# QuantEcon/dynamic_factor_models

Measured on NVIDIA H100. Metric: EM iters/sec (N=200,r=8,T=500), higher is better.
Workload: dtype f64

## Files before the change

### dynamic_factor_models_b200/csrc/dfm_kernels_fused2.cuh

```cuda
#pragma once
#include <algorithm>
#include "dfm_kernels_fused.cuh"
#ifdef DFM_EMU
struct CUtensorMap { char opaque[128]; };
#define DFM_GRID_CONSTANT
#else
#include <cuda.h>
#define DFM_GRID_CONSTANT __grid_constant__
#endif

namespace dfm {

#ifndef F2_SBS
#define F2_SBS 1
#endif
#ifndef F2_S
#define F2_S (3 / F2_SBS)
#endif
#define F2_STG (F2_SBS * 8 * F2_TS)
#ifndef F2_TC
#define F2_TC 172
#endif
#define F2_TS F2_TC
#define F2_NCW 6
#define F2_GPARTS_S 4
#define F2_GPARTS ((R == 8) ? (F2_NCW + 1) : F2_GPARTS_S)
#define F2_NRB (((F2_TC + 7) / 8 + F2_NCW - 1) / F2_NCW)
#define F2_NKC (((F2_TC + 3) / 4 + F2_NCW - 1) / F2_NCW)
static_assert(F2_TC % 16 == 4 || F2_TC % 16 == 12, "ring pitch must be 4 or 12 mod 16");
static_assert(F2_TC <= 256 && (F2_TC * 64) % 128 == 0, "TMA box / stage alignment");
#define F2_NEXS(R_) ((F2_S * F2_STG - 4 * (R_) * (R_)) / FUSED_SCR(R_))
#define F2_RTAIL(R_) (F2_S * F2_STG - 4 * (R_) * (R_))
#ifndef F2_L2WIN_PCT
#define F2_L2WIN_PCT 67
#endif

#ifndef DFM_EMU
__device__ __forceinline__ uint32_t f2_smem_u32(const void* p) { return (uint32_t)__cvta_generic_to_shared(p); }
__device__ __forceinline__ void f2_mbar_init(uint64_t* bar, int cnt) { asm volatile("mbarrier.init.shared::cta.b64 [%0], %1;" ::"r"(f2_smem_u32(bar)), "r"(cnt)); }
__device__ __forceinline__ void f2_mbar_expect(uint64_t* bar, uint32_t bytes) { asm volatile("mbarrier.arrive.expect_tx.shared::cta.b64 _, [%0], %1;" ::"r"(f2_smem_u32(bar)), "r"(bytes) : "memory"); }
__device__ __forceinline__ void f2_mbar_arrive(uint64_t* bar) { asm volatile("mbarrier.arrive.shared::cta.b64 _, [%0];" ::"r"(f2_smem_u32(bar)) : "memory"); }
__device__ __forceinline__ void f2_mbar_wait(uint64_t* bar, uint32_t phase) {
  asm volatile("{\n.reg .pred p;\nWAIT_%=:\nmbarrier.try_wait.parity.shared::cta.b64 p, [%0], %1;\n@p bra DONE_%=;\nbra WAIT_%=;\nDONE_%=:\n}" ::"r"(f2_smem_u32(bar)), "r"(phase) : "memory");
}
__device__ __forceinline__ void f2_tma_2d(void* dst, const CUtensorMap* tmap, int x, int y, uint64_t* bar, uint64_t policy) {
  asm volatile("cp.async.bulk.tensor.2d.shared::cluster.global.mbarrier::complete_tx::bytes.L2::cache_hint [%0], [%1, {%2, %3}], [%4], %5;"
               ::"r"(f2_smem_u32(dst)), "l"(reinterpret_cast<uint64_t>(tmap)), "r"(x), "r"(y), "r"(f2_smem_u32(bar)), "l"(policy) : "memory");
}

__device__ __forceinline__ int f2_round_win(const int* win, int B, int b) {
  const int G = (int)gridDim.x;
  return (b / G < B / G) ? win[0] : win[1];
}
#endif


#ifndef DFM_EMU
struct F2Ring {
  double* ring; uint64_t* full; uint64_t* empty;
  int rs; uint32_t rph; bool wrap;
  __device__ __forceinline__ void advance() { if (++rs == F2_S) { rs = 0; rph ^= 1; wrap = true; } }
  __device__ __forceinline__ void skip(long long n) { for (long long q = 0; q < n; ++q) advance(); }
};

__device__ __forceinline__ void f2_produce(F2Ring& rg, const CUtensorMap* tmap, int row0, int T, int N, bool c_outer, const int* win) {
  const int lane = threadIdx.x & 31;
  const int nsb = (N + 8 * F2_SBS - 1) / (8 * F2_SBS), nck = (T + F2_TC - 1) / F2_TC;
  const int n_out = c_outer ? nck : nsb, n_in = c_outer ? nsb : nck, nw = *win;
  const int wc = c_outer ? nck - 1 : 0, w0 = c_outer ? nsb - nw : 0, w1 = c_outer ? nsb : nw;
  uint64_t pol_win, pol_first;
  asm volatile("createpolicy.fractional.L2::evict_normal.b64 %0, 1.0;" : "=l"(pol_win));
  asm volatile("createpolicy.fractional.L2::evict_first.b64 %0, 1.0;" : "=l"(pol_first));
  for (int o = 0; o < n_out; ++o)
    for (int i = 0; i < n_in; ++i) {
      const int c = c_outer ? o : i, sb = c_outer ? i : nsb - 1 - o;
      if (rg.wrap) f2_mbar_wait(&rg.empty[rg.rs], rg.rph ^ 1);
      if (lane == 0) {
        f2_mbar_expect(&rg.full[rg.rs], (uint32_t)(F2_STG * 8));
        f2_tma_2d(rg.ring + (size_t)rg.rs * F2_STG, tmap, c * F2_TC, row0 + sb * 8 * F2_SBS, &rg.full[rg.rs],
                  (c == wc && sb >= w0 && sb < w1) ? pol_win : pol_first);
      }
      __syncwarp();
      rg.advance();
    }
}

template <int R>
__device__ __forceinline__ double f2_consume_E(F2Ring& rg, int cw, int T, int N, int Tp, int Np, double* Z, const double* Lam,
                                               const double* rinv) {
  const int lane = threadIdx.x & 31, lr = lane >> 2, lc = lane & 3;
  const int nsg = (N + 8 * F2_SBS - 1) / (8 * F2_SBS), nck = (T + F2_TC - 1) / F2_TC;
  double qacc = 0.0;
  for (int c = 0; c < nck; ++c) {
    const int len = (T - c * F2_TC < F2_TC) ? T - c * F2_TC : F2_TC;
    double d[F2_NRB][2][2];
#pragma unroll
    for (int j = 0; j < F2_NRB; ++j) { d[j][0][0] = 0.0; d[j][0][1] = 0.0; d[j][1][0] = 0.0; d[j][1][1] = 0.0; }
    for (int sg = 0; sg < nsg; ++sg) {
      f2_mbar_wait(&rg.full[rg.rs], rg.rph);
      const double* stage = rg.ring + (size_t)rg.rs * F2_STG;
#pragma unroll
      for (int sub = 0; sub < F2_SBS; ++sub) {
        const double* tile = stage + (size_t)sub * 8 * F2_TS;
        const int sb = sg * F2_SBS + sub;
        double rn[2], lm[2], av[2][F2_NRB];
#pragma unroll
        for (int kc = 0; kc < 2; ++kc) {
          const int n = sb * 8 + kc * 4 + lc;
          const bool nok = n < N;
          rn[kc] = nok ? (rinv ? rinv[n] : 1.0) : 0.0;
          lm[kc] = (nok && lr < R) ? Lam[LI(n, lr)] : 0.0;
          const double* trow = tile + (kc * 4 + lc) * F2_TS + lr;
#pragma unroll
          for (int j = 0; j < F2_NRB; ++j) {
            const int t0 = (cw + j * F2_NCW) * 8;
            av[kc][j] = (nok && t0 + lr < len) ? trow[t0] : 0.0;
          }
        }
#pragma unroll
        for (int kc = 0; kc < 2; ++kc)
#pragma unroll
          for (int j = 0; j < F2_NRB; ++j) {
            const double ar = av[kc][j] * rn[kc];
            qacc += av[kc][j] * ar;
            asm volatile("mma.sync.aligned.m8n8k4.row.col.f64.f64.f64.f64 {%0,%1}, {%2}, {%3}, {%0,%1};\n"
                         : "+d"(d[j][kc][0]), "+d"(d[j][kc][1]) : "d"(ar), "d"(lm[kc]));
          }
      }
      __syncwarp();
      if (lane == 0) f2_mbar_arrive(&rg.empty[rg.rs]);
      rg.advance();
    }
#pragma unroll
    for (int j = 0; j < F2_NRB; ++j) {
      const int tl = (cw + j * F2_NCW) * 8 + lr;
      if (tl < len) { const int t = c * F2_TC + tl; Z[ZI(t, 2 * lc)] = d[j][0][0] + d[j][1][0]; Z[ZI(t, 2 * lc + 1)] = d[j][0][1] + d[j][1][1]; }
    }
  }
  return qacc;
}

template <int R>
__device__ __forceinline__ void f2_consume_M(F2Ring& rg, int cw, int T, int N, int Tp, int Np, const double* Z, double* Lam,
                                             double* sxx, double* part) {
  const int lane = threadIdx.x & 31, lr = lane >> 2, lc = lane & 3;
  const int nsg = (N + 8 * F2_SBS - 1) / (8 * F2_SBS), nck = (T + F2_TC - 1) / F2_TC;
  double d[F2_SBS][F2_NKC][2], s2[F2_SBS];
#pragma unroll
  for (int sub = 0; sub < F2_SBS; ++sub) {
    s2[sub] = 0.0;
#pragma unroll
    for (int j = 0; j < F2_NKC; ++j) { d[sub][j][0] = 0.0; d[sub][j][1] = 0.0; }
  }
  for (int sg = nsg - 1; sg >= 0; --sg)
    for (int c = 0; c < nck; ++c) {
      f2_mbar_wait(&rg.full[rg.rs], rg.rph);
      const double* stage = rg.ring + (size_t)rg.rs * F2_STG;
      const int len = (T - c * F2_TC < F2_TC) ? T - c * F2_TC : F2_TC;
      const double* zc = Z + (size_t)lr * Tp + c * F2_TC + lc;
      double bv[F2_NKC];
#pragma unroll
      for (int j = 0; j < F2_NKC; ++j) { const int t0 = (cw + j * F2_NCW) * 4; bv[j] = (t0 + lc < len) ? zc[t0] : 0.0; }
#pragma unroll
      for (int sub = 0; sub < F2_SBS; ++sub) {
        const bool nok = (sg * F2_SBS + sub) * 8 + lr < N;
        const double* trow = stage + (size_t)sub * 8 * F2_TS + lr * F2_TS + lc;
        double av[F2_NKC];
#pragma unroll
        for (int j = 0; j < F2_NKC; ++j) { const int t0 = (cw + j * F2_NCW) * 4; av[j] = (nok && t0 + lc < len) ? trow[t0] : 0.0; }
#pragma unroll
        for (int j = 0; j < F2_NKC; ++j) {
          s2[sub] += av[j] * av[j];
          asm volatile("mma.sync.aligned.m8n8k4.row.col.f64.f64.f64.f64 {%0,%1}, {%2}, {%3}, {%0,%1};\n"
                       : "+d"(d[sub][j][0]), "+d"(d[sub][j][1]) : "d"(av[j]), "d"(bv[j]));
        }
      }
      __syncwarp();
      if (lane == 0) f2_mbar_arrive(&rg.empty[rg.rs]);
      rg.advance();
      if (c == nck - 1) {
#pragma unroll
        for (int sub = 0; sub < F2_SBS; ++sub) {
          const int sb = sg * F2_SBS + sub;
          double sq = s2[sub];
          sq += __shfl_xor_sync(0xffffffffu, sq, 1); sq += __shfl_xor_sync(0xffffffffu, sq, 2);
          double* pb = part + (size_t)(sb & 1) * F2_NCW * 72 + cw * 72;
          double t0_ = 0.0, t1_ = 0.0;
#pragma unroll
          for (int j = 0; j < F2_NKC; ++j) { t0_ += d[sub][j][0]; t1_ += d[sub][j][1]; d[sub][j][0] = 0.0; d[sub][j][1] = 0.0; }
          pb[2 * lane] = t0_; pb[2 * lane + 1] = t1_;
          if (lc == 0) pb[64 + lr] = sq;
          asm volatile("bar.sync 1, %0;" ::"n"(F2_NCW * 32) : "memory");
          const int ct = cw * 32 + lane;
          if (ct < 72) {
            const double* pp_ = part + (size_t)(sb & 1) * F2_NCW * 72 + ct;
            double tot_ = 0.0;
#pragma unroll
            for (int w_ = 0; w_ < F2_NCW; ++w_) tot_ += pp_[w_ * 72];
            if (ct < 64) {
              const int l_ = ct >> 1, h_ = ct & 1, row = l_ >> 2, col = 2 * (l_ & 3) + h_, n = sb * 8 + row;
              if (n < N && col < R) Lam[LI(n, col)] = tot_;
            } else { const int n = sb * 8 + (ct - 64); if (n < N) sxx[n] = tot_; }
          }
          s2[sub] = 0.0;
        }
      }
    }
}
#endif

#define F2_PNT_GPU ((F2_NCW + 1) * 32)
#ifdef DFM_EMU
#define F2_PSYNC() ((void)0)
#define F2_PTID 0
#define F2_PNT 1
#else
#define F2_PSYNC() asm volatile("bar.sync 2, %0;" ::"n"(F2_PNT_GPU) : "memory")
// ... 4 lines not shown
#define DFM_FUSED2_BOUNDS
#else
#define DFM_FUSED2_BOUNDS __launch_bounds__(256, 2)
#endif
template <int R>
__global__ void DFM_FUSED2_BOUNDS k_em_fused2(FusedArgs a, const DFM_GRID_CONSTANT CUtensorMap tmap) {
  DFM_SMEM(sm);
  constexpr int RR = R * R, NP = R * (R + 1) / 2;
  const int T = a.T, N = a.N;
  const int Tp = pad4mod16(T), Np = pad4mod16(N);
  double* Z = sm;
  double* Lam = Z + (size_t)FZ * Tp;
  double* rinv = Lam + (size_t)R * Np;
  double* Rv = rinv + N;
  double* sxx = Rv + N;
  double* mats = sxx + N;
  double* M = mats;            double* Q = M + RR;        double* C = Q + RR;        double* Pp = C + RR;
  double* Pi = Pp + RR;        double* Pf = Pi + RR;      double* Wm = Pf + RR;      double* G = Wm + RR;
  double* Phi = G + RR;        double* Jm = Phi + RR;     double* Pn = Jm + RR;      double* T1 = Pn + RR;
  double* T2 = T1 + RR;        double* Ps = T2 + RR;      double* Psn = Ps + RR;     double* SPall = Psn + RR;
  double* SP00 = SPall + RR;   double* SPff2 = SP00 + RR; double* SP11 = SPff2 + RR; double* Sm = SP11 + RR;
  double* S11m = Sm + RR;      double* Pfinf = S11m + RR; double* Phinf = Pfinf + RR; double* Jinf = Phinf + RR;
  double* Winf = Jinf + RR;    double* Ppinf = Winf + RR; double* IJM = Ppinf + RR;  double* Pfprev = IJM + RR;
  double* tmp = Pfprev + RR;
  double* red = tmp + 2 * R;
  double* scal = red + 40;
  int* ctl = (int*)(scal + 8);
  double* bnd = scal + 16;
  double* part = bnd;
  double* ring = bnd + (((size_t)97 * R + RR > 2 * F2_NCW * 72) ? (size_t)97 * R + RR : 2 * F2_NCW * 72);
#ifndef DFM_EMU
  ring += ((128u - (f2_smem_u32(ring) & 127u)) & 127u) / 8;
#endif
  double* gscr = a.scratch + (size_t)DFM_BX * T * FUSED_SCR(R);
#define GSC(t_) (gscr + (size_t)(t_) * FUSED_SCR(R))
#define SCRP(t_) (((t_) < F2_NEXS(R)) ? (ring + (size_t)(t_) * FUSED_SCR(R)) : (gscr + (size_t)(t_) * FUSED_SCR(R)))
#define GPS(t_) (gscr + (size_t)(t_) * FUSED_SCR(R) + 4 * RR)
#ifndef DFM_EMU
  __shared__ uint64_t fullb[F2_S], emptyb[F2_S];
  if (threadIdx.x == 0) { for (int s_ = 0; s_ < F2_S; ++s_) { f2_mbar_init(&fullb[s_], 1); f2_mbar_init(&emptyb[s_], F2_NCW); } }
  asm volatile("fence.mbarrier_init.release.cluster;" ::: "memory");
  __syncthreads();
  F2Ring rg; rg.ring = ring; rg.full = fullb; rg.empty = emptyb; rg.rs = 0; rg.rph = 0; rg.wrap = false;
#endif
  const double eps = 1e-14;

  for (int b = DFM_BX; b < a.B; b += DFM_GX) {
#ifdef DFM_EMU
    const double* X = a.X + (size_t)b * T * N;
#endif
#ifndef DFM_EMU
    if (a.ready) {
      if (threadIdx.x == 0) {
        const int* f_ = a.ready + b / a.ready_chunk; int v_ = 0;
        for (;;) { asm volatile("ld.acquire.sys.global.s32 %0, [%1];" : "=r"(v_) : "l"(f_) : "memory"); if (v_) break; __nanosleep(256); }
      }
      __syncthreads();
    }
#endif
// ... 108 lines not shown
            w_gemm<R>(T1, Pf, false, M, true);
            w_gemm<R>(Jinf, T1, false, Pi, false);
            break;
          }
          if (frozen_at < 0 && dmax <= eps * pmax) frozen_at = t;
          for (int e = DFM_LANE; e < RR; e += DFM_WSZ) Pp[e] = Pn[e];
          DFM_WSYNC();
          ++t;
        }
        const int frozen = nE < T;
        if (DFM_LANE == 0) { ctl[0] = nE; ctl[3] = frozen; }
        if (frozen) {
          w_gemm<R>(IJM, Jinf, false, M, false);
          for (int e = DFM_LANE; e < RR; e += DFM_WSZ) { int i = e / R, j = e % R; IJM[e] = ((i == j) ? 1.0 : 0.0) - IJM[e]; }
          DFM_WSYNC();
          const int n3 = T - (nE > 0 ? nE : 1), n5 = (T - 2) - (nE - 1) + 1;
          if (n3 > 0) {
            w_matpow<R>(Phi, Phinf, blk_chunk_len(n3, F2_PNT_GPU / 8), T1, T2);
            w_gemm<R>(Pp, Phi, false, Phi, false); w_gemm<R>(Pi, Pp, false, Pp, false);
            w_gemm<R>(Pf, Pi, false, Pi, false);   w_gemm<R>(Jm, Pf, false, Pf, false);
          }
          if (n5 > 0) {
            w_matpow<R>(Pn, Jinf, blk_chunk_len(n5, F2_PNT_GPU / 8), T1, T2);
            double* gl_ = GSC(T - 1);
            w_gemm<R>(T1, Pn, false, Pn, false);
            for (int e = DFM_LANE; e < RR; e += DFM_WSZ) gl_[e] = T1[e];
            w_gemm<R>(T2, T1, false, T1, false);
            for (int e = DFM_LANE; e < RR; e += DFM_WSZ) gl_[RR + e] = T2[e];
            w_gemm<R>(T1, T2, false, T2, false);
            for (int e = DFM_LANE; e < RR; e += DFM_WSZ) gl_[2 * RR + e] = T1[e];
            w_gemm<R>(T2, T1, false, T1, false);
            for (int e = DFM_LANE; e < RR; e += DFM_WSZ) gl_[3 * RR + e] = T2[e];
            DFM_WSYNC();
          }
        }
        DFM_WSYNC();
      };
      auto chain_bwd = [&]() {
        const int nE = ctl[0], frozen = ctl[3];
        int t;
        for (int e = DFM_LANE; e < RR; e += DFM_WSZ) {
          double v = frozen ? Pfinf[e] : (GSC(T - 1))[e];
          Psn[e] = v; SPall[e] = v; SPff2[e] = v; SP00[e] = 0.0; SP11[e] = 0.0;
          GPS(T - 1)[e] = v;
        }
        DFM_WSYNC();
        const int lo = frozen ? nE - 1 : T;
        int tb = -1;
        t = T - 2;
        while (t >= 0) {
          const double* pf_t = (t < nE) ? GSC(t) : Pfinf;
          const double* j_t = (t < nE - 1) ? GSC(t) + 2 * RR : Jinf;
          w_gemm<R>(T1, M, false, pf_t, false);
          w_gemm<R>(T2, T1, false, M, true);
          for (int e = DFM_LANE; e < RR; e += DFM_WSZ) T2[e] = Psn[e] - (T2[e] + Q[e]);
          DFM_WSYNC();
// ... 19 lines not shown
          if (conv) {
            tb = t;
            double cnt = (double)(t - lo);
            w_gemm<R>(T1, Ps, false, Jinf, true);
            for (int e = DFM_LANE; e < RR; e += DFM_WSZ) {
              SPall[e] += cnt * Ps[e]; SP00[e] += cnt * Ps[e];
              SPff2[e] += ((lo >= 1) ? cnt : cnt - 1.0) * Ps[e];
              SP11[e] += cnt * T1[e];
              Ppinf[e] = Ps[e];
            }
            DFM_WSYNC();
            t = lo - 1;
          } else --t;
        }
        if (DFM_LANE == 0) ctl[1] = tb;
        DFM_WSYNC();
      };
      double qacc = 0.0;
#ifdef DFM_EMU
      for (int t = 0; t < T; ++t) {
        for (int c = 0; c < FZ; ++c) Z[ZI(t, c)] = 0.0;
        for (int n = 0; n < N; ++n) {
          double x = X[(size_t)n * T + t], xr = x * rinv[n];
          qacc += x * xr;
          for (int c = 0; c < R; ++c) Z[ZI(t, c)] += xr * Lam[LI(n, c)];
        }
      }
#else
      {
        const long long nitems = (long long)((N + 8 * F2_SBS - 1) / (8 * F2_SBS)) * ((T + F2_TC - 1) / F2_TC);
        if (DFM_WARP == 0) f2_produce(rg, &tmap, b * N, T, N, true, &ctl[4]);
        else if (DFM_WARP <= F2_NCW) qacc += f2_consume_E<R>(rg, DFM_WARP - 1, T, N, Tp, Np, Z, Lam, rinv);
        else {
          rg.skip(nitems);
          chain_fwd();
        }
      }
#endif
#ifdef DFM_EMU
      chain_fwd();
      chain_bwd();
#endif
      DFM_SYNC();
      const int nE = ctl[0], frozen = ctl[3];
#ifndef DFM_EMU
      if (DFM_WARP == F2_NCW + 1) chain_bwd();
      else
#endif
      {
      {
        const int ncp = (nE < F2_NEXS(R)) ? nE : F2_NEXS(R);
        for (int e = F2_PTID; e < ncp * FUSED_SCR(R); e += F2_PNT) ring[e] = gscr[e];
        if (frozen) for (int e = F2_PTID; e < 4 * RR; e += F2_PNT) ring[F2_RTAIL(R) + e] = GSC(T - 1)[e];
      }
      for (int t = nE + F2_PTID; t < T; t += F2_PNT) {
        double bb[R], u[R];
#pragma unroll
        for (int j = 0; j < R; ++j) bb[j] = Z[ZI(t, j)];
#pragma unroll
        for (int i = 0; i < R; ++i) { double s = 0.0;
#pragma unroll
          for (int j = 0; j < R; ++j) s += Pfinf[i * R + j] * bb[j]; u[i] = s; }
#pragma unroll
        for (int i = 0; i < R; ++i) Z[ZI(t, i)] = u[i];
      }
      F2_PSYNC();
      if (DFM_WARP == 0) {
        for (int t = 0; t < nE; ++t) {
          const double* s_ = SCRP(t);
          for (int i = DFM_LANE; i < R; i += DFM_WSZ) {
            double s = 0.0;
            for (int j = 0; j < R; ++j) s += s_[i * R + j] * Z[ZI(t, j)];
            if (t >= 1) for (int j = 0; j < R; ++j) s += s_[RR + i * R + j] * Z[ZI(t - 1, j)];
            tmp[i] = s;
          }
          DFM_WSYNC();
          for (int i = DFM_LANE; i < R; i += DFM_WSZ) Z[ZI(t, i)] = tmp[i];
          DFM_WSYNC();
        }
      }
      F2_PSYNC();
      if (frozen) blk_recur<R>(Z, Tp, Phinf, Phi, Pi, bnd, (nE > 0 ? nE : 1), T - (nE > 0 ? nE : 1), +1, F2_PNT_GPU, true, Pp, Pi, Pf, Jm);
      double llp = -0.5 * qacc;
      const bool gram = frozen && nE >= 1 && nE < T;
      const bool split = gram && 2 * nE * R <= (97 * R + RR) - (F2_GPARTS + 1) * RR;
      const int tex = gram ? (split ? 0 : nE) : T;
      if (gram) {
        double* gp = bnd;
#ifndef DFM_EMU
        if (R == 8) {
          const int lr = DFM_LANE >> 2, lc = DFM_LANE & 3;
          const double* zr = Z + (size_t)lr * Tp;
          double g0 = 0.0, g1 = 0.0, h0 = 0.0, h1 = 0.0;
          for (int t0 = nE + 4 * DFM_WARP; t0 < T; t0 += 8 * (F2_NCW + 1)) {
            const int ta = t0 + lc, tb_ = t0 + 4 * (F2_NCW + 1) + lc;
            const double va = (ta < T) ? zr[ta] : 0.0, vb = (tb_ < T) ? zr[tb_] : 0.0;
            asm volatile("mma.sync.aligned.m8n8k4.row.col.f64.f64.f64.f64 {%0,%1}, {%2}, {%3}, {%0,%1};\n" : "+d"(g0), "+d"(g1) : "d"(va), "d"(va));
            asm volatile("mma.sync.aligned.m8n8k4.row.col.f64.f64.f64.f64 {%0,%1}, {%2}, {%3}, {%0,%1};\n" : "+d"(h0), "+d"(h1) : "d"(vb), "d"(vb));
          }
          gp[DFM_WARP * 64 + 2 * DFM_LANE] = g0 + h0; gp[DFM_WARP * 64 + 2 * DFM_LANE + 1] = g1 + h1;
        } else
#endif
        {
          const int nfz = T - nE, q4 = (nfz + F2_GPARTS_S - 1) / F2_GPARTS_S;
          for (int e = F2_PTID; e < F2_GPARTS * RR; e += F2_PNT) {
// ... 20 lines not shown
            zd[2 * e] = s_; zd[2 * e + 1] = Z[ZI(t, i)] - s_;
          }
        }
        if (DFM_WARP == 0) {
          for (int e = DFM_LANE; e < RR; e += DFM_WSZ) Wm[e] = Winf[e] - C[e];
          DFM_WSYNC();
          w_gemm<R>(G, Wm, false, M, false);
          w_gemm<R>(gp + F2_GPARTS * RR, M, true, G, false);
        }
        F2_PSYNC();
        for (int e = F2_PTID; e < RR; e += F2_PNT) {
          const int i = e / R, jj = e % R;
          double gf = 0.0;
#pragma unroll
          for (int q = 0; q < F2_GPARTS; ++q) gf += gp[q * RR + e];
          const double gs = gf + Z[ZI(nE - 1, i)] * Z[ZI(nE - 1, jj)] - Z[ZI(T - 1, i)] * Z[ZI(T - 1, jj)];
          llp += -0.5 * (gp[F2_GPARTS * RR + e] * gs - Winf[e] * gf);
        }
        if (F2_PTID == 0) llp += -0.5 * (double)(T - nE) * ((double)N * 1.8378770664093454835606594728112 + scal[0] + scal[1]);
        if (split) {
          const double* zd = gp + (F2_GPARTS + 1) * RR;
          for (int e = F2_PTID; e < nE * R; e += F2_PNT) {
            const int t = e / R, i = e % R;
            const double* Wt = SCRP(t) + 3 * RR;
            const double* zt = zd + 2 * (size_t)t * R;
            double cz = 0.0, g = 0.0;
#pragma unroll
            for (int j = 0; j < R; ++j) { cz += C[i * R + j] * zt[2 * j]; g += Wt[i * R + j] * zt[2 * j + 1]; }
            const double zpi = zt[2 * i], di = zt[2 * i + 1];
            llp += 0.5 * (zpi * cz + 2.0 * zpi * g + g * di);
            if (i == 0) llp += -0.5 * ((double)N * 1.8378770664093454835606594728112 + scal[0] + (SCRP(t))[5 * RR]);
          }
        }
      }
      for (int t = F2_PTID; t < tex; t += F2_PNT) {
        const double* Wt = (t < nE) ? SCRP(t) + 3 * RR : Winf;
        double ldt = (t < nE) ? (SCRP(t))[5 * RR] : scal[1];
        double zp[R], d[R];
#pragma unroll
        for (int i = 0; i < R; ++i) { double s = 0.0; if (t >= 1) {
#pragma unroll
            for (int j = 0; j < R; ++j) s += M[i * R + j] * Z[ZI(t - 1, j)]; }
          zp[i] = s; d[i] = Z[ZI(t, i)] - s; }
        double quad = 0.0;
#pragma unroll
        for (int i = 0; i < R; ++i) {
          double cz = 0.0, g = 0.0;
#pragma unroll
          for (int j = 0; j < R; ++j) { cz += C[i * R + j] * zp[j]; g += Wt[i * R + j] * d[j]; }
          quad -= zp[i] * cz + 2.0 * zp[i] * g + g * d[i];
        }
        llp += -0.5 * ((double)N * 1.8378770664093454835606594728112 + scal[0] + ldt + quad);
      }
      {
#ifndef DFM_EMU
        for (int o = 16; o > 0; o >>= 1) llp += __shfl_down_sync(0xffffffffu, llp, o);
        if (DFM_LANE == 0) red[DFM_WARP] = llp;
        F2_PSYNC();
        if (threadIdx.x == 0) { double s_ = 0.0; for (int w_ = 0; w_ <= F2_NCW; ++w_) s_ += red[w_]; scal[3] = s_; }
#else
        scal[3] = llp;
#endif
      }
      if (frozen) {
        int lo = nE - 1;
        for (int t = lo + F2_PTID; t < T - 1; t += F2_PNT) {
          double zz[R], v[R];
#pragma unroll
          for (int j = 0; j < R; ++j) zz[j] = Z[ZI(t, j)];
#pragma unroll
          for (int i = 0; i < R; ++i) { double s = 0.0;
#pragma unroll
            for (int j = 0; j < R; ++j) s += IJM[i * R + j] * zz[j]; v[i] = s; }
#pragma unroll
          for (int i = 0; i < R; ++i) Z[ZI(t, i)] = v[i];
        }
      }
      F2_PSYNC();
      if (frozen) blk_recur<R>(Z, Tp, Jinf, Pn, Pi, bnd, T - 2, (T - 2) - (nE - 1) + 1, -1, F2_PNT_GPU, true, ring + F2_RTAIL(R), ring + F2_RTAIL(R) + RR, ring + F2_RTAIL(R) + 2 * RR, ring + F2_RTAIL(R) + 3 * RR);
      if (DFM_WARP == 0) {
        const int lo = frozen ? nE - 1 : T;
        for (int t = (lo - 1 < T - 2 ? lo - 1 : T - 2); t >= 0; --t) {
          const double* j_t = SCRP(t) + 2 * RR;
          for (int i = DFM_LANE; i < R; i += DFM_WSZ) { double s = Z[ZI(t + 1, i)]; for (int j = 0; j < R; ++j) s -= M[i * R + j] * Z[ZI(t, j)]; tmp[i] = s; }
          DFM_WSYNC();
          for (int i = DFM_LANE; i < R; i += DFM_WSZ) { double s = Z[ZI(t, i)]; for (int j = 0; j < R; ++j) s += j_t[i * R + j] * tmp[j]; tmp[R + i] = s; }
          DFM_WSYNC();
          for (int i = DFM_LANE; i < R; i += DFM_WSZ) Z[ZI(t, i)] = tmp[R + i];
          DFM_WSYNC();
        }
      }
      }
      DFM_SYNC();
      const double ll = scal[3];
      auto mstep_small = [&]() {
        int* bad = &ctl[2];
#ifndef DFM_EMU
        if (R == 8) {
          const int lr = DFM_LANE >> 2, lc = DFM_LANE & 3;
          const double* zr = Z + (size_t)lr * Tp;
          double g[2][2] = {{0.0, 0.0}, {0.0, 0.0}}, h[2][2] = {{0.0, 0.0}, {0.0, 0.0}};
          for (int t0 = 0; t0 < T; t0 += 8) {
            const int ta = t0 + lc, tb_ = t0 + 4 + lc;
            const double va = (ta < T) ? zr[ta] : 0.0, vb = (tb_ < T) ? zr[tb_] : 0.0;
            const double pa = (ta >= 1 && ta < T) ? zr[ta - 1] : 0.0, pb = (tb_ < T) ? zr[tb_ - 1] : 0.0;
#define F2_DMMA(d_, a_, b_) asm volatile("mma.sync.aligned.m8n8k4.row.col.f64.f64.f64.f64 {%0,%1}, {%2}, {%3}, {%0,%1};\n" : "+d"((d_)[0]), "+d"((d_)[1]) : "d"(a_), "d"(b_))
// ... 20 lines not shown
        w_sym<R>(T1);
        w_inv<R>(G, T1, tmp, bad);
        for (int e = DFM_LANE; e < RR; e += DFM_WSZ) {
          int i = e / R, j = e % R;
          Pp[e] = Sm[e] - Z[ZI(T - 1, i)] * Z[ZI(T - 1, j)] + SP00[e];
          Pi[e] = Sm[e] - Z[ZI(0, i)] * Z[ZI(0, j)] + SPff2[e];
          Pf[e] = S11m[e] + SP11[e];
        }
        DFM_WSYNC();
        w_sym<R>(Pp);
        w_inv<R>(Wm, Pp, tmp, bad);
        w_gemm<R>(Phi, Pf, false, Wm, false);
        w_gemm<R>(Pn, Phi, false, Pf, true);
        for (int e = DFM_LANE; e < RR; e += DFM_WSZ) Pn[e] = (Pi[e] - Pn[e]) / (double)(T - 1);
        DFM_WSYNC();
        w_sym<R>(Pn);
      };
#ifdef DFM_EMU
      for (int n = 0; n < N; ++n) {
        double s2 = 0.0, acc[R];
        for (int c = 0; c < R; ++c) acc[c] = 0.0;
        for (int t = 0; t < T; ++t) { double x = X[(size_t)n * T + t]; s2 += x * x; for (int c = 0; c < R; ++c) acc[c] += x * Z[ZI(t, c)]; }
        for (int c = 0; c < R; ++c) Lam[LI(n, c)] = acc[c];
        sxx[n] = s2;
      }
#else
      {
        asm volatile("fence.proxy.async.shared::cta;" ::: "memory");
        __syncthreads();
        const long long nitems = (long long)((N + 8 * F2_SBS - 1) / (8 * F2_SBS)) * ((T + F2_TC - 1) / F2_TC);
        if (DFM_WARP == 0) f2_produce(rg, &tmap, b * N, T, N, false, &ctl[4]);
        else if (DFM_WARP <= F2_NCW) f2_consume_M<R>(rg, DFM_WARP - 1, T, N, Tp, Np, Z, Lam, sxx, part);
        else {
          rg.skip(nitems);
          mstep_small();
        }
      }
#endif
#ifdef DFM_EMU
      mstep_small();
#endif
      DFM_SYNC();
      DFM_SYNC();
      for (int n = DFM_TID; n < N; n += DFM_NT) {
        double sx[R], lam[R];
#pragma unroll
        for (int c = 0; c < R; ++c) sx[c] = Lam[LI(n, c)];
        double q1 = 0.0, q2 = 0.0;
#pragma unroll
        for (int i = 0; i < R; ++i) { double s = 0.0;
#pragma unroll
          for (int j = 0; j < R; ++j) s += G[i * R + j] * sx[j]; lam[i] = s; q1 += s * sx[i]; }
#pragma unroll
        for (int i = 0; i < R; ++i) { double s = 0.0;
#pragma unroll
          for (int j = 0; j < R; ++j) s += T1[i * R + j] * lam[j]; q2 += lam[i] * s; }
#pragma unroll
        for (int c = 0; c < R; ++c) Lam[LI(n, c)] = lam[c];
        Rv[n] = (sxx[n] - 2.0 * q1 + q2) / (double)T;
      }
      DFM_SYNC();
      for (int e = DFM_TID; e < RR; e += DFM_NT) { M[e] = Phi[e]; Q[e] = Pn[e]; }
      if (DFM_TID == 0) a.loglik[(size_t)b * a.max_iter + it] = ll;
      DFM_SYNC();
      if (ctl[2] || !(ll == ll)) { status = 3; ++it; break; }
      bool conv = (it >= 1) && fabs(ll - ll_prev) <= a.tol * 0.5 * (fabs(ll) + fabs(ll_prev));
      ll_prev = ll;
      if (conv) { ++it; break; }
    }
    for (int e = DFM_TID; e < N * R; e += DFM_NT) { int i = e % N, c = e / N; a.Lam[(size_t)b * N * R + e] = Lam[LI(i, c)]; }
    for (int e = DFM_TID; e < N; e += DFM_NT) a.R[(size_t)b * N + e] = Rv[e];
    for (int e = DFM_TID; e < RR; e += DFM_NT) {
      int i = e % R, j = e / R;
      a.A[(size_t)b * RR + e] = M[i * R + j]; a.Q[(size_t)b * RR + e] = Q[i * R + j];
    }
    for (int e = DFM_TID; e < T * R; e += DFM_NT) { int t = e % T, c = e / T; a.Fs[(size_t)b * T * R + e] = Z[ZI(t, c)]; }
    {
      const int nE = ctl[0], tb = ctl[1], frozen = ctl[3];
      const int lo = frozen ? nE - 1 : T;
      for (int e = DFM_TID; e < T * NP; e += DFM_NT) {
        int t = e % T, pe = e / T;
        int i = 0; while ((i + 1) * (i + 2) / 2 <= pe) ++i;
        int j = pe - i * (i + 1) / 2;
        bool in_frozen = frozen && tb >= 0 && t >= lo && t < tb;
        double v = in_frozen ? Ppinf[i * R + j] : GPS(t)[i * R + j];
        a.PsF[(size_t)b * T * NP + e] = v;
      }
    }
    if (DFM_TID == 0) { a.iters[b] = it > a.max_iter ? a.max_iter : it; a.status[b] = status; }
#ifndef DFM_EMU
    if (a.done) __threadfence_system();
#endif
    DFM_SYNC();
#ifndef DFM_EMU
    if (a.done && threadIdx.x == 0) *(volatile int*)(a.done + b) = 1;
#endif
  }
}

#undef SCRP
#undef GSC
#undef GPS
struct AlsFusedArgs {
  const double* Xs;
  double* F;
  double* Lam;
  AlsState* st;
  int B, T, N;
  double tol;
  long long max_iter;
  int l2_win[2];
};

template <int R>
__global__ void DFM_FUSED2_BOUNDS k_als_fused2(AlsFusedArgs a, const DFM_GRID_CONSTANT CUtensorMap tmap) {
  DFM_SMEM(sm);
  constexpr int RR = R * R;
  const int T = a.T, N = a.N;
  const int Tp = pad4mod16(T), Np = pad4mod16(N);
  double* Z = sm;
  double* Lam = Z + (size_t)FZ * Tp;
  double* sxx = Lam + (size_t)R * Np;
  double* FtF = sxx + N;  double* Gi = FtF + RR;  double* LtL = Gi + RR;  double* Hi = LtL + RR;
// ... 3 lines not shown
  double* part = red + 48;
  double* ring = part + 2 * F2_NCW * 72;
#ifndef DFM_EMU
  ring += ((128u - (f2_smem_u32(ring) & 127u)) & 127u) / 8;
  __shared__ uint64_t fullb[F2_S], emptyb[F2_S];
  if (threadIdx.x == 0) { for (int s_ = 0; s_ < F2_S; ++s_) { f2_mbar_init(&fullb[s_], 1); f2_mbar_init(&emptyb[s_], F2_NCW); } }
  asm volatile("fence.mbarrier_init.release.cluster;" ::: "memory");
  __syncthreads();
  F2Ring rg; rg.ring = ring; rg.full = fullb; rg.empty = emptyb; rg.rs = 0; rg.rph = 0; rg.wrap = false;
  const long long nitems = (long long)((N + 8 * F2_SBS - 1) / (8 * F2_SBS)) * ((T + F2_TC - 1) / F2_TC);
#endif
  for (int b = DFM_BX; b < a.B; b += DFM_GX) {
#ifdef DFM_EMU
    const double* X = a.Xs + (size_t)b * T * N;
#endif
    for (int e = DFM_TID; e < FZ * Tp; e += DFM_NT) Z[e] = 0.0;
    DFM_SYNC();
    for (int e = DFM_TID; e < T * R; e += DFM_NT) { int t = e % T, c = e / T; Z[ZI(t, c)] = a.F[(size_t)b * T * R + e]; }
    if (DFM_TID == 0) ctl[0] = 0;
#ifndef DFM_EMU
    if (DFM_TID == 0) ctl[1] = f2_round_win(a.l2_win, a.B, b);
#endif
    DFM_SYNC();
    double ssr = 0.0, ssr_old = 0.0;
    long long it = 0;
    int status = 0;
    while (it < a.max_iter) {
      for (int e = DFM_TID; e < RR; e += DFM_NT) {
        int i = e / R, j = e % R; double s = 0.0;
        for (int t = 0; t < T; ++t) s += Z[ZI(t, i)] * Z[ZI(t, j)];
        FtF[e] = s;
      }
      DFM_SYNC();
      if (DFM_WARP == 0) w_inv<R>(Gi, FtF, tmp, &ctl[0]);
#ifdef DFM_EMU
      for (int n = 0; n < N; ++n) {
        double s2 = 0.0, acc[R];
        for (int c = 0; c < R; ++c) acc[c] = 0.0;
        for (int t = 0; t < T; ++t) { double x = X[(size_t)n * T + t]; s2 += x * x; for (int c = 0; c < R; ++c) acc[c] += x * Z[ZI(t, c)]; }
        for (int c = 0; c < R; ++c) Lam[LI(n, c)] = acc[c];
        sxx[n] = s2;
      }
#else
      if (DFM_WARP == 0) f2_produce(rg, &tmap, b * N, T, N, false, &ctl[1]);
      else if (DFM_WARP <= F2_NCW) f2_consume_M<R>(rg, DFM_WARP - 1, T, N, Tp, Np, Z, Lam, sxx, part);
      else rg.skip(nitems);
#endif
      DFM_SYNC();
      for (int n = DFM_TID; n < N; n += DFM_NT) {
        double sx[R], lam[R];
#pragma unroll
        for (int c = 0; c < R; ++c) sx[c] = Lam[LI(n, c)];
#pragma unroll
        for (int i = 0; i < R; ++i) { double s = 0.0;
#pragma unroll
          for (int j = 0; j < R; ++j) s += Gi[i * R + j] * sx[j]; lam[i] = s; }
#pragma unroll
        for (int c = 0; c < R; ++c) Lam[LI(n, c)] = lam[c];
      }
      DFM_SYNC();
      for (int e = DFM_TID; e < RR; e += DFM_NT) {
        int i = e / R, j = e % R; double s = 0.0;
        for (int n = 0; n < N; ++n) s += Lam[LI(n, i)] * Lam[LI(n, j)];
        LtL[e] = s;
      }
      DFM_SYNC();
      if (DFM_WARP == 0) w_inv<R>(Hi, LtL, tmp, &ctl[0]);
      double tssp = 0.0;
#ifdef DFM_EMU
      for (int t = 0; t < T; ++t) {
        for (int c = 0; c < FZ; ++c) Z[ZI(t, c)] = 0.0;
        for (int n = 0; n < N; ++n) { double x = X[(size_t)n * T + t]; tssp += x * x; for (int c = 0; c < R; ++c) Z[ZI(t, c)] += x * Lam[LI(n, c)]; }
      }
#else
      if (DFM_WARP == 0) f2_produce(rg, &tmap, b * N, T, N, true, &ctl[1]);
      else if (DFM_WARP <= F2_NCW) tssp += f2_consume_E<R>(rg, DFM_WARP - 1, T, N, Tp, Np, Z, Lam, nullptr);
      else rg.skip(nitems);
#endif
      DFM_SYNC();
      double bf = 0.0;
      for (int t = DFM_TID; t < T; t += DFM_NT) {
        double bb[R], f[R];
#pragma unroll
        for (int j = 0; j < R; ++j) bb[j] = Z[ZI(t, j)];
#pragma unroll
        for (int i = 0; i < R; ++i) { double s = 0.0;
#pragma unroll
          for (int j = 0; j < R; ++j) s += Hi[i * R + j] * bb[j]; f[i] = s; bf += s * bb[i]; }
#pragma unroll
        for (int i = 0; i < R; ++i) Z[ZI(t, i)] = f[i];
      }
      bf = block_sum(bf, red);
      tssp = block_sum(tssp, red);
      ssr_old = ssr; ssr = tssp - bf;
      ++it;
      if (ctl[0]) { status = 3; break; }
      if (!(fabs(ssr_old - ssr) >= a.tol * (double)T * (double)N)) break;
      if (it >= a.max_iter) { status = 4; break; }
    }
    for (int e = DFM_TID; e < T * R; e += DFM_NT) { int t = e % T, c = e / T; a.F[(size_t)b * T * R + e] = Z[ZI(t, c)]; }
    for (int e = DFM_TID; e < N * R; e += DFM_NT) { int i = e % N, c = e / N; a.Lam[(size_t)b * N * R + e] = Lam[LI(i, c)]; }
    if (DFM_TID == 0) { a.st[b].ssr_old = ssr_old; a.st[b].ssr = ssr; a.st[b].iters = (int)it; a.st[b].done = 1; a.st[b].status = status; }
    DFM_SYNC();
  }
}

template <int R>
inline size_t als_fused2_smem_doubles(int T, int N) {
  return (size_t)FZ * pad4mod16(T) + (size_t)R * pad4mod16(N) + (size_t)N + 4 * (size_t)R * R + 2 * R + 48 +
         2 * F2_NCW * 72 + (size_t)F2_S * F2_STG + 26;
}

template <int R>
inline size_t fused2_smem_doubles(int T, int N) {
  return (size_t)FZ * pad4mod16(T) + (size_t)R * pad4mod16(N) + 3 * (size_t)N + 30 * (size_t)R * R + 2 * R + 40 + 8 + 8 +
         std::max((size_t)97 * R + (size_t)R * R, (size_t)2 * F2_NCW * 72) + (size_t)F2_S * F2_STG + 26;
}

// ... 2 lines not shown
```

Measured before the change: 1.732 million.

## Prefetch next pass TMA stages early and compute data sum-of-squares once

The TMA producer can now issue a sub-range of items, so the first F2_S ring stages of the next E or M pass are launched before the intervening small serial work (inverses, Lam/Z updates, Kalman scratch), hiding pipeline fill latency. The per-iteration sum of squares of X (sxx/tssp/qacc) is computed only on the first iteration and reused afterwards. The Kalman scratch no longer lives in the TMA ring: its data moves to dedicated smem buffers or is read from global memory with L1 prefetch, so the ring can be refilled early. This reduces the per-iteration FLOPs and removes bubbles, but reads scratch from global memory instead of shared memory and adds more complex ring phase bookkeeping.

```diff
diff --git a/dynamic_factor_models_b200/csrc/dfm_kernels_fused2.cuh b/dynamic_factor_models_b200/csrc/dfm_kernels_fused2.cuh
--- a/dynamic_factor_models_b200/csrc/dfm_kernels_fused2.cuh
+++ b/dynamic_factor_models_b200/csrc/dfm_kernels_fused2.cuh
@@ -30,7 +30,6 @@
 static_assert(F2_TC % 16 == 4 || F2_TC % 16 == 12, "ring pitch must be 4 or 12 mod 16");
 static_assert(F2_TC <= 256 && (F2_TC * 64) % 128 == 0, "TMA box / stage alignment");
 #define F2_NEXS(R_) ((F2_S * F2_STG - 4 * (R_) * (R_)) / FUSED_SCR(R_))
-#define F2_RTAIL(R_) (F2_S * F2_STG - 4 * (R_) * (R_))
 #ifndef F2_L2WIN_PCT
 #define F2_L2WIN_PCT 67
 #endif
@@ -63,7 +62,8 @@
   __device__ __forceinline__ void skip(long long n) { for (long long q = 0; q < n; ++q) advance(); }
 };
 
-__device__ __forceinline__ void f2_produce(F2Ring& rg, const CUtensorMap* tmap, int row0, int T, int N, bool c_outer, const int* win) {
+__device__ __forceinline__ void f2_produce(F2Ring& rg, const CUtensorMap* tmap, int row0, int T, int N, bool c_outer, const int* win,
+                                           int q0 = 0, int q1 = 1 << 30) {
   const int lane = threadIdx.x & 31;
   const int nsb = (N + 8 * F2_SBS - 1) / (8 * F2_SBS), nck = (T + F2_TC - 1) / F2_TC;
   const int n_out = c_outer ? nck : nsb, n_in = c_outer ? nsb : nck, nw = *win;
@@ -71,21 +71,22 @@
   uint64_t pol_win, pol_first;
   asm volatile("createpolicy.fractional.L2::evict_normal.b64 %0, 1.0;" : "=l"(pol_win));
   asm volatile("createpolicy.fractional.L2::evict_first.b64 %0, 1.0;" : "=l"(pol_first));
-  for (int o = 0; o < n_out; ++o)
-    for (int i = 0; i < n_in; ++i) {
-      const int c = c_outer ? o : i, sb = c_outer ? i : nsb - 1 - o;
-      if (rg.wrap) f2_mbar_wait(&rg.empty[rg.rs], rg.rph ^ 1);
-      if (lane == 0) {
-        f2_mbar_expect(&rg.full[rg.rs], (uint32_t)(F2_STG * 8));
-        f2_tma_2d(rg.ring + (size_t)rg.rs * F2_STG, tmap, c * F2_TC, row0 + sb * 8 * F2_SBS, &rg.full[rg.rs],
-                  (c == wc && sb >= w0 && sb < w1) ? pol_win : pol_first);
-      }
-      __syncwarp();
-      rg.advance();
-    }
-}
-
-template <int R>
+  if (q1 > n_out * n_in) q1 = n_out * n_in;
+  for (int q = q0, o = q0 / n_in, i = q0 % n_in; q < q1; ++q) {
+    const int c = c_outer ? o : i, sb = c_outer ? i : nsb - 1 - o;
+    if (rg.wrap) f2_mbar_wait(&rg.empty[rg.rs], rg.rph ^ 1);
+    if (lane == 0) {
+      f2_mbar_expect(&rg.full[rg.rs], (uint32_t)(F2_STG * 8));
+      f2_tma_2d(rg.ring + (size_t)rg.rs * F2_STG, tmap, c * F2_TC, row0 + sb * 8 * F2_SBS, &rg.full[rg.rs],
+                (c == wc && sb >= w0 && sb < w1) ? pol_win : pol_first);
+    }
+    __syncwarp();
+    rg.advance();
+    if (++i == n_in) { i = 0; ++o; }
+  }
+}
+
+template <int R, bool SQ>
 __device__ __forceinline__ double f2_consume_E(F2Ring& rg, int cw, int T, int N, int Tp, int Np, double* Z, const double* Lam,
                                                const double* rinv) {
   const int lane = threadIdx.x & 31, lr = lane >> 2, lc = lane & 3;
@@ -122,7 +123,7 @@
 #pragma unroll
           for (int j = 0; j < F2_NRB; ++j) {
             const double ar = av[kc][j] * rn[kc];
-            qacc += av[kc][j] * ar;
+            if (SQ) qacc += av[kc][j] * ar;
             asm volatile("mma.sync.aligned.m8n8k4.row.col.f64.f64.f64.f64 {%0,%1}, {%2}, {%3}, {%0,%1};\n"
                          : "+d"(d[j][kc][0]), "+d"(d[j][kc][1]) : "d"(ar), "d"(lm[kc]));
           }
@@ -140,7 +141,7 @@
   return qacc;
 }
 
-template <int R>
+template <int R, bool SXX>
 __device__ __forceinline__ void f2_consume_M(F2Ring& rg, int cw, int T, int N, int Tp, int Np, const double* Z, double* Lam,
                                              double* sxx, double* part) {
   const int lane = threadIdx.x & 31, lr = lane >> 2, lc = lane & 3;
@@ -170,7 +171,7 @@
         for (int j = 0; j < F2_NKC; ++j) { const int t0 = (cw + j * F2_NCW) * 4; av[j] = (nok && t0 + lc < len) ? trow[t0] : 0.0; }
 #pragma unroll
         for (int j = 0; j < F2_NKC; ++j) {
-          s2[sub] += av[j] * av[j];
+          if (SXX) s2[sub] += av[j] * av[j];
           asm volatile("mma.sync.aligned.m8n8k4.row.col.f64.f64.f64.f64 {%0,%1}, {%2}, {%3}, {%0,%1};\n"
                        : "+d"(d[sub][j][0]), "+d"(d[sub][j][1]) : "d"(av[j]), "d"(bv[j]));
         }
@@ -182,17 +183,17 @@
 #pragma unroll
         for (int sub = 0; sub < F2_SBS; ++sub) {
           const int sb = sg * F2_SBS + sub;
-          double sq = s2[sub];
-          sq += __shfl_xor_sync(0xffffffffu, sq, 1); sq += __shfl_xor_sync(0xffffffffu, sq, 2);
+          double sq = 0.0;
+          if (SXX) { sq = s2[sub]; sq += __shfl_xor_sync(0xffffffffu, sq, 1); sq += __shfl_xor_sync(0xffffffffu, sq, 2); }
           double* pb = part + (size_t)(sb & 1) * F2_NCW * 72 + cw * 72;
           double t0_ = 0.0, t1_ = 0.0;
 #pragma unroll
           for (int j = 0; j < F2_NKC; ++j) { t0_ += d[sub][j][0]; t1_ += d[sub][j][1]; d[sub][j][0] = 0.0; d[sub][j][1] = 0.0; }
           pb[2 * lane] = t0_; pb[2 * lane + 1] = t1_;
-          if (lc == 0) pb[64 + lr] = sq;
+          if (SXX && lc == 0) pb[64 + lr] = sq;
           asm volatile("bar.sync 1, %0;" ::"n"(F2_NCW * 32) : "memory");
           const int ct = cw * 32 + lane;
-          if (ct < 72) {
+          if (ct < (SXX ? 72 : 64)) {
             const double* pp_ = part + (size_t)(sb & 1) * F2_NCW * 72 + ct;
             double tot_ = 0.0;
 #pragma unroll
@@ -243,7 +244,8 @@
   double* SP00 = SPall + RR;   double* SPff2 = SP00 + RR; double* SP11 = SPff2 + RR; double* Sm = SP11 + RR;
   double* S11m = Sm + RR;      double* Pfinf = S11m + RR; double* Phinf = Pfinf + RR; double* Jinf = Phinf + RR;
   double* Winf = Jinf + RR;    double* Ppinf = Winf + RR; double* IJM = Ppinf + RR;  double* Pfprev = IJM + RR;
-  double* tmp = Pfprev + RR;
+  double* Jl2 = Pfprev + RR;   double* Jl4 = Jl2 + RR;
+  double* tmp = Jl4 + RR;
   double* red = tmp + 2 * R;
   double* scal = red + 40;
   int* ctl = (int*)(scal + 8);
@@ -255,7 +257,6 @@
 #endif
   double* gscr = a.scratch + (size_t)DFM_BX * T * FUSED_SCR(R);
 #define GSC(t_) (gscr + (size_t)(t_) * FUSED_SCR(R))
-#define SCRP(t_) (((t_) < F2_NEXS(R)) ? (ring + (size_t)(t_) * FUSED_SCR(R)) : (gscr + (size_t)(t_) * FUSED_SCR(R)))
 #define GPS(t_) (gscr + (size_t)(t_) * FUSED_SCR(R) + 4 * RR)
 #ifndef DFM_EMU
   __shared__ uint64_t fullb[F2_S], emptyb[F2_S];
@@ -410,16 +411,8 @@
           }
           if (n5 > 0) {
             w_matpow<R>(Pn, Jinf, blk_chunk_len(n5, F2_PNT_GPU / 8), T1, T2);
-            double* gl_ = GSC(T - 1);
-            w_gemm<R>(T1, Pn, false, Pn, false);
-            for (int e = DFM_LANE; e < RR; e += DFM_WSZ) gl_[e] = T1[e];
-            w_gemm<R>(T2, T1, false, T1, false);
-            for (int e = DFM_LANE; e < RR; e += DFM_WSZ) gl_[RR + e] = T2[e];
-            w_gemm<R>(T1, T2, false, T2, false);
-            for (int e = DFM_LANE; e < RR; e += DFM_WSZ) gl_[2 * RR + e] = T1[e];
-            w_gemm<R>(T2, T1, false, T1, false);
-            for (int e = DFM_LANE; e < RR; e += DFM_WSZ) gl_[3 * RR + e] = T2[e];
-            DFM_WSYNC();
+            w_gemm<R>(Jl2, Pn, false, Pn, false);  w_gemm<R>(Jl4, Jl2, false, Jl2, false);
+            w_gemm<R>(Sm, Jl4, false, Jl4, false); w_gemm<R>(S11m, Sm, false, Sm, false);
           }
         }
         DFM_WSYNC();
@@ -485,16 +478,18 @@
         for (int c = 0; c < FZ; ++c) Z[ZI(t, c)] = 0.0;
         for (int n = 0; n < N; ++n) {
           double x = X[(size_t)n * T + t], xr = x * rinv[n];
-          qacc += x * xr;
+          if (it == 0) qacc += x * xr;
           for (int c = 0; c < R; ++c) Z[ZI(t, c)] += xr * Lam[LI(n, c)];
         }
       }
 #else
       {
         const long long nitems = (long long)((N + 8 * F2_SBS - 1) / (8 * F2_SBS)) * ((T + F2_TC - 1) / F2_TC);
-        if (DFM_WARP == 0) f2_produce(rg, &tmap, b * N, T, N, true, &ctl[4]);
-        else if (DFM_WARP <= F2_NCW) qacc += f2_consume_E<R>(rg, DFM_WARP - 1, T, N, Tp, Np, Z, Lam, rinv);
-        else {
+        if (DFM_WARP == 0) f2_produce(rg, &tmap, b * N, T, N, true, &ctl[4], it > 0 ? F2_S : 0);
+        else if (DFM_WARP <= F2_NCW) {
+          if (it == 0) qacc = f2_consume_E<R, true>(rg, DFM_WARP - 1, T, N, Tp, Np, Z, Lam, rinv);
+          else f2_consume_E<R, false>(rg, DFM_WARP - 1, T, N, Tp, Np, Z, Lam, rinv);
+        } else {
           rg.skip(nitems);
           chain_fwd();
         }
@@ -511,11 +506,16 @@
       else
 #endif
       {
+#ifndef DFM_EMU
+      if (DFM_WARP == 0) f2_produce(rg, &tmap, b * N, T, N, false, &ctl[4], 0, F2_S);
       {
-        const int ncp = (nE < F2_NEXS(R)) ? nE : F2_NEXS(R);
-        for (int e = F2_PTID; e < ncp * FUSED_SCR(R); e += F2_PNT) ring[e] = gscr[e];
-        if (frozen) for (int e = F2_PTID; e < 4 * RR; e += F2_PNT) ring[F2_RTAIL(R) + e] = GSC(T - 1)[e];
-      }
+        constexpr int NL = (3 * RR + 15) / 16 + 1;
+        for (int e = F2_PTID; e < nE * NL; e += F2_PNT) {
+          const int t = e / NL, k = e % NL;
+          asm volatile("prefetch.global.L1 [%0];" ::"l"(__cvta_generic_to_global(GSC(t) + ((16 * k < 3 * RR) ? 16 * k : 3 * RR - 1))));
+        }
+      }
+#endif
       for (int t = nE + F2_PTID; t < T; t += F2_PNT) {
         double bb[R], u[R];
 #pragma unroll
@@ -530,7 +530,7 @@
       F2_PSYNC();
       if (DFM_WARP == 0) {
         for (int t = 0; t < nE; ++t) {
-          const double* s_ = SCRP(t);
+          const double* s_ = GSC(t);
           for (int i = DFM_LANE; i < R; i += DFM_WSZ) {
             double s = 0.0;
             for (int j = 0; j < R; ++j) s += s_[i * R + j] * Z[ZI(t, j)];
@@ -544,6 +544,7 @@
       }
       F2_PSYNC();
       if (frozen) blk_recur<R>(Z, Tp, Phinf, Phi, Pi, bnd, (nE > 0 ? nE : 1), T - (nE > 0 ? nE : 1), +1, F2_PNT_GPU, true, Pp, Pi, Pf, Jm);
+      if (it > 0) for (int n = F2_PTID; n < N; n += F2_PNT) qacc += sxx[n] * rinv[n];
       double llp = -0.5 * qacc;
       const bool gram = frozen && nE >= 1 && nE < T;
       const bool split = gram && 2 * nE * R <= (97 * R + RR) - (F2_GPARTS + 1) * RR;
@@ -610,20 +611,20 @@
           const double* zd = gp + (F2_GPARTS + 1) * RR;
           for (int e = F2_PTID; e < nE * R; e += F2_PNT) {
             const int t = e / R, i = e % R;
-            const double* Wt = SCRP(t) + 3 * RR;
+            const double* Wt = GSC(t) + 3 * RR;
             const double* zt = zd + 2 * (size_t)t * R;
             double cz = 0.0, g = 0.0;
 #pragma unroll
             for (int j = 0; j < R; ++j) { cz += C[i * R + j] * zt[2 * j]; g += Wt[i * R + j] * zt[2 * j + 1]; }
             const double zpi = zt[2 * i], di = zt[2 * i + 1];
             llp += 0.5 * (zpi * cz + 2.0 * zpi * g + g * di);
-            if (i == 0) llp += -0.5 * ((double)N * 1.8378770664093454835606594728112 + scal[0] + (SCRP(t))[5 * RR]);
+            if (i == 0) llp += -0.5 * ((double)N * 1.8378770664093454835606594728112 + scal[0] + (GSC(t))[5 * RR]);
           }
         }
       }
       for (int t = F2_PTID; t < tex; t += F2_PNT) {
-        const double* Wt = (t < nE) ? SCRP(t) + 3 * RR : Winf;
-        double ldt = (t < nE) ? (SCRP(t))[5 * RR] : scal[1];
+        const double* Wt = (t < nE) ? GSC(t) + 3 * RR : Winf;
+        double ldt = (t < nE) ? (GSC(t))[5 * RR] : scal[1];
         double zp[R], d[R];
 #pragma unroll
         for (int i = 0; i < R; ++i) { double s = 0.0; if (t >= 1) {
@@ -665,11 +666,11 @@
         }
       }
       F2_PSYNC();
-      if (frozen) blk_recur<R>(Z, Tp, Jinf, Pn, Pi, bnd, T - 2, (T - 2) - (nE - 1) + 1, -1, F2_PNT_GPU, true, ring + F2_RTAIL(R), ring + F2_RTAIL(R) + RR, ring + F2_RTAIL(R) + 2 * RR, ring + F2_RTAIL(R) + 3 * RR);
+      if (frozen) blk_recur<R>(Z, Tp, Jinf, Pn, Pi, bnd, T - 2, (T - 2) - (nE - 1) + 1, -1, F2_PNT_GPU, true, Jl2, Jl4, Sm, S11m);
       if (DFM_WARP == 0) {
         const int lo = frozen ? nE - 1 : T;
         for (int t = (lo - 1 < T - 2 ? lo - 1 : T - 2); t >= 0; --t) {
-          const double* j_t = SCRP(t) + 2 * RR;
+          const double* j_t = GSC(t) + 2 * RR;
           for (int i = DFM_LANE; i < R; i += DFM_WSZ) { double s = Z[ZI(t + 1, i)]; for (int j = 0; j < R; ++j) s -= M[i * R + j] * Z[ZI(t, j)]; tmp[i] = s; }
           DFM_WSYNC();
           for (int i = DFM_LANE; i < R; i += DFM_WSZ) { double s = Z[ZI(t, i)]; for (int j = 0; j < R; ++j) s += j_t[i * R + j] * tmp[j]; tmp[R + i] = s; }
@@ -736,16 +737,16 @@
         for (int c = 0; c < R; ++c) acc[c] = 0.0;
         for (int t = 0; t < T; ++t) { double x = X[(size_t)n * T + t]; s2 += x * x; for (int c = 0; c < R; ++c) acc[c] += x * Z[ZI(t, c)]; }
         for (int c = 0; c < R; ++c) Lam[LI(n, c)] = acc[c];
-        sxx[n] = s2;
+        if (it == 0) sxx[n] = s2;
       }
 #else
       {
-        asm volatile("fence.proxy.async.shared::cta;" ::: "memory");
-        __syncthreads();
         const long long nitems = (long long)((N + 8 * F2_SBS - 1) / (8 * F2_SBS)) * ((T + F2_TC - 1) / F2_TC);
-        if (DFM_WARP == 0) f2_produce(rg, &tmap, b * N, T, N, false, &ctl[4]);
-        else if (DFM_WARP <= F2_NCW) f2_consume_M<R>(rg, DFM_WARP - 1, T, N, Tp, Np, Z, Lam, sxx, part);
-        else {
+        if (DFM_WARP == 0) f2_produce(rg, &tmap, b * N, T, N, false, &ctl[4], F2_S);
+        else if (DFM_WARP <= F2_NCW) {
+          if (it == 0) f2_consume_M<R, true>(rg, DFM_WARP - 1, T, N, Tp, Np, Z, Lam, sxx, part);
+          else f2_consume_M<R, false>(rg, DFM_WARP - 1, T, N, Tp, Np, Z, Lam, sxx, part);
+        } else {
           rg.skip(nitems);
           mstep_small();
         }
@@ -755,6 +756,12 @@
       mstep_small();
 #endif
       DFM_SYNC();
+      const bool fail = ctl[2] || !(ll == ll);
+      const bool conv = !fail && (it >= 1) && fabs(ll - ll_prev) <= a.tol * 0.5 * (fabs(ll) + fabs(ll_prev));
+#ifndef DFM_EMU
+      if (DFM_WARP == 0 && !fail && !conv && it + 1 < a.max_iter)
+        f2_produce(rg, &tmap, b * N, T, N, true, &ctl[4], 0, F2_S);
+#endif
       DFM_SYNC();
       for (int n = DFM_TID; n < N; n += DFM_NT) {
         double sx[R], lam[R];
@@ -777,8 +784,7 @@
       for (int e = DFM_TID; e < RR; e += DFM_NT) { M[e] = Phi[e]; Q[e] = Pn[e]; }
       if (DFM_TID == 0) a.loglik[(size_t)b * a.max_iter + it] = ll;
       DFM_SYNC();
-      if (ctl[2] || !(ll == ll)) { status = 3; ++it; break; }
-      bool conv = (it >= 1) && fabs(ll - ll_prev) <= a.tol * 0.5 * (fabs(ll) + fabs(ll_prev));
+      if (fail) { status = 3; ++it; break; }
       ll_prev = ll;
       if (conv) { ++it; break; }
     }
@@ -812,7 +818,6 @@
   }
 }
 
-#undef SCRP
 #undef GSC
 #undef GPS
 struct AlsFusedArgs {
@@ -862,7 +867,7 @@
     if (DFM_TID == 0) ctl[1] = f2_round_win(a.l2_win, a.B, b);
 #endif
     DFM_SYNC();
-    double ssr = 0.0, ssr_old = 0.0;
+    double ssr = 0.0, ssr_old = 0.0, tss = 0.0;
     long long it = 0;
     int status = 0;
     while (it < a.max_iter) {
@@ -879,14 +884,24 @@
         for (int c = 0; c < R; ++c) acc[c] = 0.0;
         for (int t = 0; t < T; ++t) { double x = X[(size_t)n * T + t]; s2 += x * x; for (int c = 0; c < R; ++c) acc[c] += x * Z[ZI(t, c)]; }
         for (int c = 0; c < R; ++c) Lam[LI(n, c)] = acc[c];
-        sxx[n] = s2;
+        if (it == 0) sxx[n] = s2;
       }
 #else
-      if (DFM_WARP == 0) f2_produce(rg, &tmap, b * N, T, N, false, &ctl[1]);
-      else if (DFM_WARP <= F2_NCW) f2_consume_M<R>(rg, DFM_WARP - 1, T, N, Tp, Np, Z, Lam, sxx, part);
-      else rg.skip(nitems);
-#endif
-      DFM_SYNC();
+      if (DFM_WARP == 0) f2_produce(rg, &tmap, b * N, T, N, false, &ctl[1], it > 0 ? F2_S : 0);
+      else if (DFM_WARP <= F2_NCW) {
+        if (it == 0) f2_consume_M<R, true>(rg, DFM_WARP - 1, T, N, Tp, Np, Z, Lam, sxx, part);
+        else f2_consume_M<R, false>(rg, DFM_WARP - 1, T, N, Tp, Np, Z, Lam, sxx, part);
+      } else rg.skip(nitems);
+#endif
+      DFM_SYNC();
+#ifndef DFM_EMU
+      if (DFM_WARP == 0) f2_produce(rg, &tmap, b * N, T, N, true, &ctl[1], 0, F2_S);
+#endif
+      if (it == 0) {
+        double s_ = 0.0;
+        for (int n = DFM_TID; n < N; n += DFM_NT) s_ += sxx[n];
+        tss = block_sum(s_, red);
+      }
       for (int n = DFM_TID; n < N; n += DFM_NT) {
         double sx[R], lam[R];
 #pragma unroll
@@ -906,15 +921,14 @@
       }
       DFM_SYNC();
       if (DFM_WARP == 0) w_inv<R>(Hi, LtL, tmp, &ctl[0]);
-      double tssp = 0.0;
 #ifdef DFM_EMU
       for (int t = 0; t < T; ++t) {
         for (int c = 0; c < FZ; ++c) Z[ZI(t, c)] = 0.0;
-        for (int n = 0; n < N; ++n) { double x = X[(size_t)n * T + t]; tssp += x * x; for (int c = 0; c < R; ++c) Z[ZI(t, c)] += x * Lam[LI(n, c)]; }
+        for (int n = 0; n < N; ++n) { double x = X[(size_t)n * T + t]; for (int c = 0; c < R; ++c) Z[ZI(t, c)] += x * Lam[LI(n, c)]; }
       }
 #else
-      if (DFM_WARP == 0) f2_produce(rg, &tmap, b * N, T, N, true, &ctl[1]);
-      else if (DFM_WARP <= F2_NCW) tssp += f2_consume_E<R>(rg, DFM_WARP - 1, T, N, Tp, Np, Z, Lam, nullptr);
+      if (DFM_WARP == 0) f2_produce(rg, &tmap, b * N, T, N, true, &ctl[1], F2_S);
+      else if (DFM_WARP <= F2_NCW) f2_consume_E<R, false>(rg, DFM_WARP - 1, T, N, Tp, Np, Z, Lam, nullptr);
       else rg.skip(nitems);
 #endif
       DFM_SYNC();
@@ -931,9 +945,12 @@
         for (int i = 0; i < R; ++i) Z[ZI(t, i)] = f[i];
       }
       bf = block_sum(bf, red);
-      tssp = block_sum(tssp, red);
-      ssr_old = ssr; ssr = tssp - bf;
+      ssr_old = ssr; ssr = tss - bf;
       ++it;
+#ifndef DFM_EMU
+      if (DFM_WARP == 0 && !ctl[0] && fabs(ssr_old - ssr) >= a.tol * (double)T * (double)N && it < a.max_iter)
+        f2_produce(rg, &tmap, b * N, T, N, false, &ctl[1], 0, F2_S);
+#endif
       if (ctl[0]) { status = 3; break; }
       if (!(fabs(ssr_old - ssr) >= a.tol * (double)T * (double)N)) break;
       if (it >= a.max_iter) { status = 4; break; }
```

Result: faster. 1.783 million, median of 6 (+2.9%).
